# nmdp-bioinformatics/py-graph-imputation

Measured on AMD Instinct MI355X. Metric: imputed subjects/sec (whole node), 5-locus CAU graph, higher is better.
Workload: dtype f64; 1 GPU; BASELINE configs[1]: CAU 5-locus graph, 10k synthetic fully-typed subjects; 10000 subjects per step and GPU, seed=rank; graph_nodes=35411, populations=1

## Files before the change

### include/grim_hip.h

```cpp
#ifndef GRIM_HIP_H
#define GRIM_HIP_H

#include <stddef.h>
#include <stdint.h>

#ifdef __cplusplus
extern "C" {
#endif

#define GRIM_MAXL 5
#define GRIM_ABITS 12
#define GRIM_KEY_GRAPH_ORDER 60
#define GRIM_MAXPH 16
#define GRIM_MAXPOP 64
#define GRIM_TOPCAP 128
#define GRIM_MAXLADDER 64
#define GRIM_MAXROWS 8

typedef struct grim_ctx grim_ctx;
typedef struct grim_graph grim_graph;
typedef struct grim_batch grim_batch;

grim_ctx *grim_create(int device_id);
void grim_destroy(grim_ctx *ctx);
// ... 190 lines not shown
  const char *mask_ids;
  const uint8_t *mask_fixed;
  uint32_t n_masks;
} grim_stream_opts;

typedef struct {
  uint64_t lines, subjects, chunks, reruns;
  uint64_t unsupported;
  double wall_s;
  double tokenize_cpu_s, format_cpu_s, write_cpu_s;
  double device_s;
  double kernel_ms[7];
  uint64_t counters[4];
  uint64_t text_bytes[7];
  uint64_t bytes_h2d, bytes_d2h;
} grim_stream_stats;

grim_stream *grim_stream_open(grim_ctx *ctx, const grim_graph *g, const grim_dict *dict, const grim_params *prm,
                              const grim_prior_spec *priors, const char *const *pop_names, uint32_t n_pops,
                              const grim_stream_opts *opts);
int grim_stream_write(grim_stream *s, const char *text, uint64_t len);
int grim_stream_write_borrowed(grim_stream *s, const char *text, uint64_t len);
int grim_stream_write_text(grim_stream *s, const char *text, uint64_t len);
int grim_stream_write_file(grim_stream *s, const char *path);
int grim_stream_segment(grim_stream *s, uint64_t next_line_offset);
uint32_t grim_stream_n_segments(const grim_stream *s);
int grim_stream_segment_end(const grim_stream *s, uint32_t k, uint64_t out[7]);
int grim_stream_segment_wait(grim_stream *s, uint32_t k, uint64_t sizes[7]);
int grim_stream_segment_place(grim_stream *s, uint32_t k, const uint64_t base[6]);
int64_t grim_chunk_offsets(const char *path, uint32_t chunk_lines, uint64_t **out);
void grim_free(void *p);
uint32_t grim_default_threads(void);
int grim_stream_finish(grim_stream *s);
const char *grim_stream_error(const grim_stream *s);
const char *grim_stream_text(grim_stream *s, int which, uint64_t *len);
int grim_stream_get_stats(const grim_stream *s, grim_stream_stats *out);
int grim_stream_devtok_lines(const grim_stream *s, uint64_t *offered, uint64_t *handed_back);
uint32_t grim_tokname_hash(const char *name, uint32_t len);
uint64_t grim_stream_n_unsupported(const grim_stream *s);
int grim_stream_unsupported(const grim_stream *s, uint64_t k, uint64_t *line, uint32_t *reason, const char **id, uint32_t *id_len);
typedef struct {
  uint64_t first_line;
  uint32_t n_lines;
  const uint8_t *kinds;
  const grim_subject_result *res;
  const grim_row *rows;
  void *chunk;
// ... 108 lines not shown
```

### py-graph-imputation_amd/csrc/grim_engine.hip

```cpp
#include <hip/hip_runtime.h>
#include <hip/hip_ext.h>
#include <stdio.h>
#include <stdlib.h>
#include <string.h>
#include <algorithm>
#include <atomic>
#include <mutex>
#include <string>
#include <vector>

#include "grim_plan_a.h"
#include "grim_plan_b.h"
#include "grim_small.h"
#include "grim_medium.h"
#include "grim_mid.h"
#include "grim_tables.h"
#include "grim_tokdev.h"
#include "grim_em.h"
#include "grim_refresh.h"
#include "grim_marginal.h"
#include "grim_match.h"
#include "grim_search.h"
#include "grim_engine_internal.h"
#include "grim_host_internal.h"
// ... 1352 lines not shown
  }
  HIPCHK(hipEventRecord(b->ev_done, c->stream), c, -1);
  b->enqueued = true;
  return 0;
}

static int read_phase_times(grim_batch *b) {
  for (int p = 0; p < PH_COUNT; ++p)
    if (b->launched >> p & 1) HIPCHK(hipEventElapsedTime(&b->ms[p], b->ev[p][0], b->ev[p][1]), b->ctx, -1);
  b->launched = 0;
  return 0;
}

static inline uint32_t planb_count(const uint32_t *q) { return q[GRIM_Q_NEXT] + q[GRIM_Q_NEXT_HEAVY]; }

int engine_batch_wait(grim_batch *b) {
  if (!b) return -1;
  grim_ctx *c = b->ctx;
  use_device(c->device);
  DevArgs &A = b->a;
  if (!b->enqueued) {
    set_err(c, "engine_batch_wait: nothing in flight");
    return -1;
  }
  b->enqueued = false;
  b->ran_ok = false;
  HIPCHK(hipEventSynchronize(b->ev_done), c, -1);
  if (read_phase_times(b) != 0) return -1;
  uint32_t q[GRIM_NQ];
  auto read_queue = [&] { memcpy(q, b->hstate + GRIM_NCTR, sizeof(q)); };
  read_queue();
  const bool run_b = A.prm.planb && planb_count(q) > 0;
  if (run_b || stage2_pending(q) > 0) {
    {
      std::lock_guard<std::mutex> lk(c->run_mu);
      if (bind_scratch(b) != 0) return -1;
      if (run_b) {
        uint32_t grid = b->n_slots < planb_count(q) ? b->n_slots : planb_count(q);
        launch(b, PH_PLAN_B, grim_plan_b_kernel, dim3(grid), dim3(GRIM_WG), A);
        if (hipGetLastError() != hipSuccess) {
          set_err(c, "grim_batch_run: plan-B launch failed");
          return -1;
        }
      }
      enqueue_tables(b);
      launch(b, PH_NONE, grim_finish_kernel, dim3(1), dim3(GRIM_WG), A.counters, b->hstate, 0u, 1);
      HIPCHK(hipGetLastError(), c, -1);
      HIPCHK(hipEventRecord(b->ev_done, c->stream), c, -1);
    }
    HIPCHK(hipEventSynchronize(b->ev_done), c, -1);
    if (read_phase_times(b) != 0) return -1;
    read_queue();
  }
  if (b->timing) {
    for (int p = 0; p < PH_COUNT; ++p) b->acc_ms[p] += b->ms[p];
    b->n_timed++;
  }
  static const int dbg_classes = env_int("GRIM_DEBUG_CLASSES", 0);
  if (dbg_classes)
    fprintf(stderr, "grim classes: mid-size kernel took %u, handed %u to the general kernel\n"
            "grim classes: small %u medium %u general %u | medium->general %u (+%u heavier), to plan B %u (+%u heavy) | table items %u one-wave, %u bigger (%u work units), %u pair records; workgroup merge: %u items (%u with an overflowed bucket), up to %u pairs; workgroup split: %u items | stage 1 %s\n",
            q[GRIM_Q_MID_WORK], q[GRIM_Q_MID], b->n_small, b->n_medium, b->n_general, q[GRIM_Q_BAIL], q[GRIM_Q_BAIL_HEAVY], q[GRIM_Q_NEXT], q[GRIM_Q_NEXT_HEAVY], q[GRIM_Q_T1], q[GRIM_Q_T2],
            q[GRIM_Q_TUNITS], q[GRIM_Q_POOL], q[GRIM_Q_DBG_MERGE_WG], q[GRIM_Q_DBG_MERGE_OVF], q[GRIM_Q_DBG_MERGE_MAX], q[GRIM_Q_DBG_SPLIT_WG],
            b->graph_state == 1 ? "replayed as a hipGraph" : "launched directly");
  memcpy(b->counters, b->hstate, sizeof(b->counters));
// ... 157 lines not shown
  }();
  return on;
}
int engine_batch_fetch_issue(grim_batch *b) {
  if (!b) return -1;
  const bool ct = ct_on() != 0;
  if (ct) {
    b->ct_slot = (int)(g_ct_k.fetch_add(1) & 63);
    (void)hipEventRecord(g_ct_ev[0][b->ct_slot], b->ctx->copy_stream);
  }
  if (batch_fetch_on(b, 0, b->n_subj, nullptr, b->ctx->copy_stream, false) != 0) return -1;
  if (ct) (void)hipEventRecord(g_ct_ev[1][b->ct_slot], b->ctx->copy_stream);
  if (ct || !b->fetch_hsa) HIPCHK(hipEventRecord(b->ev_copy, b->ctx->copy_stream), b->ctx, -1);
  return 0;
}
int engine_batch_fetch_wait(grim_batch *b) {
  if (!b) return -1;
  use_device(b->ctx->device);
  if (b->fetch_hsa) {
    b->fetch_hsa = false;
    if (grim_sdma_wait(b->ctx->sdma, b->sdma_job) != 0) {
      set_err(b->ctx, "engine_batch_fetch: the SDMA copy of the results failed");
      return -1;
    }
    return 0;
  }
  HIPCHK(hipEventSynchronize(b->ev_copy), b->ctx, -1);
  if (ct_on() && b->ct_slot >= 0) {
    float ms = 0;
    if (hipEventElapsedTime(&ms, g_ct_ev[0][b->ct_slot], g_ct_ev[1][b->ct_slot]) == hipSuccess) { g_ct_ns += (uint64_t)(ms * 1e6); ++g_ct_n; }
    b->ct_slot = -1;
  }
  return 0;
}
extern "C" int grim_batch_results(grim_batch *b, grim_subject_result *res, grim_row *rows) {
  if (!b) return -1;
  grim_ctx *c = b->ctx;
  use_device(c->device);
  if (b->n_subj) HIPCHK(hipMemcpy(res, b->a.res, sizeof(grim_subject_result) * (size_t)b->n_subj, hipMemcpyDeviceToHost), c, -1);
  if (b->rows_used) HIPCHK(hipMemcpy(rows, b->a.rows, sizeof(grim_row) * (size_t)b->rows_used, hipMemcpyDeviceToHost), c, -1);
  return 0;
}
// ... 1302 lines not shown
```

### py-graph-imputation_amd/csrc/grim_engine_internal.h

```cpp
#pragma once
#include <stdint.h>

#include "../../include/grim_hip.h"
#include "grim_layout.h"
#include "grim_tok.h"

struct EnginePlan {
  uint32_t n_subj;
  uint64_t tok_cap;
  uint64_t text_cap;
};

struct EngineHost {
  grim_subject *subj;
  uint16_t *tok;
  SmallRec *small;
  uint32_t *order_s, *order_m, *order_g;
  grim_subject_result *res;
  grim_row *rows;
  LineRec *lines;
  uint8_t *text;
};

struct EngineLoad {
// ... 5 lines not shown
  uint32_t dev_lo, dev_hi;
  uint64_t text_bytes;
};

grim_batch *engine_batch_create(grim_ctx *ctx, const grim_graph *g, const grim_params *p, uint64_t row_limit, const EnginePlan *plan);
int engine_batch_plan(grim_batch *b, const EnginePlan *plan);
const EngineHost *engine_batch_host(grim_batch *b);
uint32_t engine_small_stride(const grim_params *p);
uint64_t engine_rows_per_subject(const grim_params *p, uint32_t n_pops);
int engine_batch_load(grim_batch *b, const EngineLoad *ld);
int engine_batch_fetch(grim_batch *b, uint32_t res_lo, uint32_t res_hi, grim_row *rows_dst);
uint64_t engine_bytes_moved(const grim_batch *b, int dir);
void engine_set_error(grim_ctx *ctx, const char *msg);
void engine_batch_recycle(grim_batch *b);
int engine_batch_fetch_issue(grim_batch *b);
int engine_batch_fetch_wait(grim_batch *b);
int engine_batch_upload_done(grim_batch *b);
int engine_batch_enqueue(grim_batch *b);
int engine_batch_wait(grim_batch *b);
struct DictSnap;
typedef struct grim_devdict grim_devdict;
grim_devdict *engine_devdict_create(grim_ctx *ctx, const DictSnap *snap);
void engine_devdict_free(grim_devdict *d);
void engine_batch_set_dict(grim_batch *b, const grim_devdict *d);
uint32_t engine_batch_irregular(const grim_batch *b);
uint32_t engine_graph_order_bad(const grim_graph *g);
uint64_t engine_batch_pool_want(const grim_batch *b);
void engine_batch_hint_pool(grim_batch *b, uint64_t records);
int engine_batch_grow_pool(grim_batch *b, uint64_t max_records);
int engine_batch_grow_rows(grim_batch *b, uint64_t max_rows);
uint64_t engine_batch_row_limit(const grim_batch *b);
void engine_batch_hint_rows(grim_batch *b, uint64_t rows);
```

### py-graph-imputation_amd/csrc/grim_host.cpp

```cpp
#include <stdint.h>
#include <stdlib.h>
#include <string.h>

#include <algorithm>
#include <charconv>
#include <cmath>
#include <mutex>
#include <string>
#include <string_view>
#include <thread>
#include <unordered_map>
#include <vector>

#include "../../include/grim_hip.h"

#include "grim_host_internal.h"

extern "C" grim_dict *grim_dict_create(uint32_t n_loci) {
  if (n_loci == 0 || n_loci > GRIM_MAXL) return nullptr;
  grim_dict *d = new grim_dict();
  d->n_loci = n_loci;
  d->locus_name.resize(n_loci);
  d->ids.resize(n_loci);
  d->names.resize(n_loci);
// ... 1113 lines not shown
  if (len) *len = t->t[which].size();
  return t->t[which].data();
}

extern "C" void grim_text_free(grim_text *t) { delete t; }

extern "C" int grim_format_double(double x, char *buf, int cap) {
  char b[48];
  char *e = py_float_to(x, b);
  const int n = (int)(e - b);
  if (n + 1 > cap) return -1;
  memcpy(buf, b, (size_t)n);
  buf[n] = 0;
  return n;
}
```

### py-graph-imputation_amd/csrc/grim_sdma.cpp

```cpp
#include "grim_sdma.h"

#include <hsa/hsa.h>
#include <hsa/hsa_ext_amd.h>
#include <stdio.h>
#include <stdlib.h>
#include <string.h>

#include <vector>

struct GrimSdma {
  hsa_agent_t gpu, cpu;
  hsa_amd_sdma_engine_id_t engine;
  uint64_t spin_ticks;
  uint32_t rec, avail;
  bool pinned_by_env;
};

namespace {
struct Agents {
  std::vector<hsa_agent_t> gpus, cpus;
};
hsa_status_t collect(hsa_agent_t a, void *data) {
  Agents *A = (Agents *)data;
  hsa_device_type_t t;
// ... 139 lines not shown
}

int grim_sdma_d2h_issue(GrimSdma *s, uint64_t job, void *dst_host, const void *src_dev, size_t bytes) {
  if (!s || !job) return -1;
  hsa_signal_t sig;
  sig.handle = job;
  hsa_signal_store_relaxed(sig, 1);
  const hsa_status_t st = hsa_amd_memory_async_copy_on_engine(dst_host, s->cpu, src_dev, s->gpu, bytes, 0, nullptr, sig, s->engine, true);
  if (st != HSA_STATUS_SUCCESS) {
    hsa_signal_store_relaxed(sig, 0);
    return -1;
  }
  return 0;
}

int grim_sdma_wait(GrimSdma *s, uint64_t job) {
  if (!s || !job) return -1;
  hsa_signal_t sig;
  sig.handle = job;
  hsa_signal_value_t v = hsa_signal_wait_scacquire(sig, HSA_SIGNAL_CONDITION_LT, 1, s->spin_ticks, HSA_WAIT_STATE_ACTIVE);
  while (v >= 1) v = hsa_signal_wait_scacquire(sig, HSA_SIGNAL_CONDITION_LT, 1, UINT64_MAX, HSA_WAIT_STATE_BLOCKED);
  return v < 0 ? -1 : 0;
}
```

### py-graph-imputation_amd/csrc/grim_sdma.h

```cpp
#pragma once
#include <stddef.h>
#include <stdint.h>

struct GrimSdma;

GrimSdma *grim_sdma_open(const char *hip_pci_bus_id, int hip_device_ordinal, const char **why);
void grim_sdma_close(GrimSdma *s);
uint32_t grim_sdma_engine(const GrimSdma *s);
uint32_t grim_sdma_pick(GrimSdma *s, void *dst_host, const void *src_dev, size_t bytes, char *report, size_t report_len);

int grim_sdma_job_create(GrimSdma *s, uint64_t *job);
void grim_sdma_job_destroy(GrimSdma *s, uint64_t job);
int grim_sdma_d2h_issue(GrimSdma *s, uint64_t job, void *dst_host, const void *src_dev, size_t bytes);
int grim_sdma_wait(GrimSdma *s, uint64_t job);
```

### py-graph-imputation_amd/csrc/grim_stream.cpp

```cpp
#include <errno.h>
#include <execinfo.h>
#include <fcntl.h>
#include <signal.h>
#include <sched.h>
#include <hip/hip_runtime_api.h>
#include <stdint.h>
#include <stdio.h>
#include <stdlib.h>
#include <string.h>
#include <sys/stat.h>
#include <sys/types.h>
#include <unistd.h>
#if defined(__x86_64__)
#include <immintrin.h>
#endif

#include <algorithm>
#include <atomic>
#include <chrono>
#include <condition_variable>
#include <deque>
#include <memory>
#include <mutex>
#include <string>
// ... 205 lines not shown
    char *dst = nullptr;
    size_t n = 0;
    std::vector<uint32_t> nl;
    uint32_t n_nl = 0;
  };
  std::vector<std::thread> copiers;
  std::vector<CopyJob> copy_jobs;
  std::atomic<uint64_t> copy_ticket{0}, copy_np_gen{0};
  std::mutex copy_mu;
  std::condition_variable cv_copyjob;
  std::atomic<uint64_t> copy_gen{0};
  std::atomic<int> copy_left{0};
  bool copy_stop = false;
  uint32_t avg_line = 128;
  std::thread dev_thread, copy_thread, fetch_thread;
  std::deque<Chunk *> copy_q, fetch_q;
  std::condition_variable cv_copy, cv_fetch;
  uint64_t next_device = 0, next_commit = 0, next_record = 0, n_done = 0;

  int fd[6] = {-1, -1, -1, -1, -1, -1};
  uint64_t file_pos[7] = {0, 0, 0, 0, 0, 0, 0};
  std::vector<std::pair<char *, size_t>> mem[7];
  std::string joined[7];
  bool joined_ok[7] = {false, false, false, false, false, false, false};

  struct Unsup {
    uint64_t line;
    uint32_t reason;
    std::string id;
  };
// ... 317 lines not shown
    Chunk *c = nullptr;
    {
      std::unique_lock<std::mutex> lk(s->mu);
      for (;;) {
        if (s->stop || s->failed) return;
        c = s->by_index(s->next_device);
        if (c && c->state == CH_TOKENIZED) break;
        c = nullptr;
        if (loaded) break;
        s->cv_dev.wait(lk);
      }
      if (c) ++s->next_device;
    }
    if (!c && loaded && !eager) {
      const auto w0 = Clock::now();
      for (int spin = 0;; ++spin) {
        if (engine_batch_upload_done(loaded->batch)) break;
        if ((spin & 7) == 7) {
          if (secs(w0, Clock::now()) > 200e-6) break;
          std::unique_lock<std::mutex> lk(s->mu, std::try_to_lock);
          if (lk.owns_lock()) {
            if (s->stop || s->failed) return;
            Chunk *n = s->by_index(s->next_device);
            if (n && n->state == CH_TOKENIZED) {
              c = n;
              ++s->next_device;
              break;
            }
          }
        }
// ... 33 lines not shown
      Chunk *l = loaded;
      loaded = nullptr;
      if (!launch(l, 0)) return;
    }
    if (c) {
      if (c->n_dev_subjects && rc == 0) {
        loaded = c;
      } else if (!launch(c, rc)) {
        return;
      }
    }
  }
}

static void copy_loop(grim_stream *s) {
  for (;;) {
    Chunk *c = nullptr;
    {
      std::unique_lock<std::mutex> lk(s->mu);
      for (;;) {
        if (s->stop || s->failed) return;
        if (!s->copy_q.empty()) {
          c = s->copy_q.front();
          s->copy_q.pop_front();
          break;
        }
        s->cv_copy.wait(lk);
      }
    }
    const auto t0 = Clock::now();
    int rc = 0;
    PartStats ps;
    if (c->n_dev_subjects) {
      if (c->in_flight) {
        c->in_flight = false;
        const int wrc = engine_batch_wait(c->batch);
        tl_note(c, 5);
        auto lb = [](const std::vector<uint32_t> &v, uint32_t x) { return (size_t)(std::lower_bound(v.begin(), v.end(), x) - v.begin()); };
        const size_t rng[4] = {0, lb(c->os, c->n_lines), 0, lb(c->om, c->n_lines)};
        rc = finish_part(s, c, 0, c->n_lines, true, wrc, rng, (uint32_t)c->og_sorted.size(), ps);
      } else {
        rc = device_part_sync(s, c, 0, c->n_lines, true, ps);
      }
      if (rc == 0 && !c->extra_rows.empty()) c->rows = c->extra_rows.data();
    }
    const auto t1 = Clock::now();
    g_dbg_ns[2] += (uint64_t)(secs(t0, t1) * 1e9);
    bool issued = false, fetched_ok = true;
    if (rc == 0 && c->n_dev_subjects && c->fetch_pending && c->extra_rows.empty()) {
      fetched_ok = engine_batch_fetch_issue(c->batch) == 0;
      issued = fetched_ok;
// ... 10 lines not shown
        s->fail(std::string(rc != 0 ? "device stage failed: " : "device stage failed: copying the results to the host: ") + (e ? e : ""));
        return;
      }
      if (issued) {
        s->fetch_q.push_back(c);
        s->cv_fetch.notify_all();
      } else {
        c->state = CH_DEVICE_DONE;
      }
    }
    if (!issued) enqueue_format(s, c);
  }
}

static void fetch_loop(grim_stream *s) {
  for (;;) {
    Chunk *c = nullptr;
    {
      std::unique_lock<std::mutex> lk(s->mu);
      for (;;) {
        if (s->stop || s->failed) return;
        if (!s->fetch_q.empty()) {
          c = s->fetch_q.front();
          s->fetch_q.pop_front();
          break;
        }
        s->cv_fetch.wait(lk);
      }
    }
    const auto t0 = Clock::now();
    const bool ok = engine_batch_fetch_wait(c->batch) == 0;
    tl_note(c, 7);
    g_dbg_ns[3] += (uint64_t)(secs(t0, Clock::now()) * 1e9);
    {
      std::lock_guard<std::mutex> lk(s->mu);
      if (!ok) {
        const char *e = grim_last_error(s->ctx);
        s->fail(std::string("device stage failed: copying the results to the host: ") + (e ? e : ""));
        return;
      }
      c->rows = engine_batch_host(c->batch)->rows;
      c->state = CH_DEVICE_DONE;
    }
    enqueue_format(s, c);
  }
}
// ... 223 lines not shown
  uint32_t k = 0;
  for (size_t i = 0; i < n; ++i) {
    dst[i] = src[i];
    if (src[i] == '\n') nl[k++] = (uint32_t)i;
  }
  return k;
}

static constexpr size_t COPY_PIECES = 64;
static void copy_pieces(grim_stream *s) {
  for (;;) {
    const uint64_t t = s->copy_ticket.fetch_add(1, std::memory_order_acq_rel);
    const uint64_t ng = s->copy_np_gen.load(std::memory_order_acquire);
    const uint32_t k = (uint32_t)t;
    if ((ng >> 32) != (t >> 32) || k >= (uint32_t)ng) return;
    grim_stream::CopyJob &job = s->copy_jobs[k];
    tl_dbg[0] = k; tl_dbg[1] = (uint64_t)job.dst; tl_dbg[2] = (uint64_t)job.src; tl_dbg[3] = job.n; tl_dbg[4] = (uint64_t)job.nl.data();
    tl_dbg[5] = job.nl.size(); tl_dbg[6] = t; tl_dbg[7] = ng;
    job.n_nl = copy_and_mark(job.dst, job.src, job.n, job.nl.data());
    s->copy_left.fetch_sub(1, std::memory_order_release);
  }
}

static void copier_loop(grim_stream *s, size_t) {
  uint64_t seen = 0;
  for (;;) {
    {
      uint64_t gen = s->copy_gen.load(std::memory_order_acquire);
      if (gen == seen) {
        const auto t0 = Clock::now();
        for (int spin = 0; gen == seen; ++spin) {
          if ((spin & 63) == 63 && secs(t0, Clock::now()) > 250e-6) break;
#if defined(__x86_64__)
          __builtin_ia32_pause();
#endif
          gen = s->copy_gen.load(std::memory_order_acquire);
        }
      }
      if (gen == seen) {
        std::unique_lock<std::mutex> lk(s->copy_mu);
        s->cv_copyjob.wait(lk, [&] { return s->copy_stop || s->copy_gen.load(std::memory_order_acquire) != seen; });
        if (s->copy_stop) return;
        gen = s->copy_gen.load(std::memory_order_acquire);
      }
      seen = gen;
    }
    copy_pieces(s);
  }
}

static Chunk *acquire_chunk(grim_stream *s) {
  std::unique_lock<std::mutex> lk(s->mu);
// ... 245 lines not shown
        for (size_t k = 0; k < parts; ++k) {
          const size_t o = std::min<size_t>(blk, k * per), e = std::min<size_t>(blk, (k + 1) * per);
          grim_stream::CopyJob &j = s->copy_jobs[k];
          j.src = text + a + o;
          j.dst = as_view ? nullptr : c->text.data() + base + o;
          j.n = e - o;
          j.n_nl = 0;
          if (j.nl.size() < j.n + 64) j.nl.resize(j.n + 64);
        }
        const uint64_t blk_no = (s->copy_gen.load(std::memory_order_relaxed) + 1) & 0xFFFFFFFFull;
        s->copy_np_gen.store(blk_no << 32 | (uint64_t)parts, std::memory_order_release);
        s->copy_left.store((int)parts);
        s->copy_ticket.store(blk_no << 32, std::memory_order_release);
        s->copy_gen.fetch_add(1, std::memory_order_release);
      }
      s->cv_copyjob.notify_all();
      copy_pieces(s);
      while (s->copy_left.load(std::memory_order_acquire) > 0) std::this_thread::yield();
      const auto tr2 = Clock::now();
      g_dbg_ns[8] += (uint64_t)(secs(tr1, tr2) * 1e9);
      used = blk;
      bool full = false;
      for (size_t q = 0; q < parts && !full; ++q) {
        const grim_stream::CopyJob &j = s->copy_jobs[q];
        const uint64_t po = std::min<size_t>(blk, q * per);
        const uint32_t take = std::min<uint32_t>(j.n_nl, want - got);
        uint32_t ln = c->n_lines + got;
        uint32_t first = s->granule - ln % s->granule;
        for (uint32_t i = first; i <= take; i += s->granule)
          if (ln + i < s->chunk_lines) c->mark_off.push_back(base + po + j.nl[i - 1] + 1);
        got += take;
// ... 201 lines not shown
  }
  if (len) *len = s->joined[which].size();
  return s->joined[which].data();
}

extern "C" int grim_stream_get_stats(const grim_stream *s, grim_stream_stats *out) {
  if (!s || !out) return -1;
  {
    std::lock_guard<std::mutex> lk(const_cast<grim_stream *>(s)->mu);
    *out = s->st;
  }
  out->tokenize_cpu_s = s->tok_ns.load() * 1e-9;
  out->format_cpu_s = s->fmt_ns.load() * 1e-9;
  out->write_cpu_s = s->wr_ns.load() * 1e-9;
  out->unsupported = s->unsupported.size();
  out->bytes_h2d = engine_bytes_moved(nullptr, 0);
  out->bytes_d2h = engine_bytes_moved(nullptr, 1);
  return 0;
}

extern "C" int grim_stream_devtok_lines(const grim_stream *s, uint64_t *offered, uint64_t *handed_back) {
  if (!s) return -1;
  if (offered) *offered = s->offered.load();
  if (handed_back) *handed_back = s->handed_back.load();
  return 0;
}

extern "C" uint64_t grim_stream_n_unsupported(const grim_stream *s) { return s ? s->unsupported.size() : 0; }

extern "C" int grim_stream_unsupported(const grim_stream *s, uint64_t k, uint64_t *line, uint32_t *reason, const char **id, uint32_t *id_len) {
// ... 31 lines not shown
  }
}

extern "C" int grim_stream_release_records(grim_stream *s, grim_stream_records *rec) {
  if (!s || !rec || !rec->chunk) return -1;
  Chunk *c = (Chunk *)rec->chunk;
  std::lock_guard<std::mutex> lk(s->mu);
  c->records_released = true;
  tl_note(c, 9);
  tl_close(c);
  rec->chunk = nullptr;
  release_if_done(s, c);
  return 0;
}

extern "C" uint32_t grim_default_threads(void) {
  unsigned cores = 0;
  cpu_set_t set;
  CPU_ZERO(&set);
  if (sched_getaffinity(0, sizeof(set), &set) == 0) cores = (unsigned)CPU_COUNT(&set);
  if (!cores) cores = std::max(1u, std::thread::hardware_concurrency());
  unsigned ranks = 1;
  const char *lw = getenv("LOCAL_WORLD_SIZE");
  if (!lw || atoi(lw) <= 0) lw = getenv("WORLD_SIZE");
  if (lw && atoi(lw) > 0) ranks = (unsigned)atoi(lw);
  unsigned nt = cores / ranks;
  if (nt < 1) nt = 1;
  if (nt > 32) nt = 32;
  return nt;
}

static void segv_backtrace(int sig, siginfo_t *si, void *) {
  void *frames[48];
  const int n = backtrace(frames, 48);
  char buf[512];
  const int m = snprintf(buf, sizeof(buf), "grim: SIGSEGV at address %p; copy job: k=%llu dst=%llx src=%llx n=%llu nl=%llx nl_size=%llu ticket=%llx np_gen=%llx\n"
                         "native frames of the faulting thread:\n", si ? si->si_addr : nullptr, (unsigned long long)tl_dbg[0], (unsigned long long)tl_dbg[1],
                         (unsigned long long)tl_dbg[2], (unsigned long long)tl_dbg[3], (unsigned long long)tl_dbg[4], (unsigned long long)tl_dbg[5],
                         (unsigned long long)tl_dbg[6], (unsigned long long)tl_dbg[7]);
  (void)!write(2, buf, (size_t)m);
  backtrace_symbols_fd(frames, n, 2);
  signal(sig, SIG_DFL);
// ... 49 lines not shown
      p += n + 1;
    }
    s->have_masks = true;
  } else if (opts->mask_ids) {
    s->have_masks = true;
  }
  s->rule.small_ok = (n_pops == 1) && prm->opt_threshold > 1 && !getenv("GRIM_NO_SMALL") && engine_graph_order_bad(g) == 0;
  s->rule.medium_ok = !getenv("GRIM_NO_MEDIUM") && engine_graph_order_bad(g) == 0;
  s->rule.medium_max_cost = getenv("GRIM_MEDIUM_MAXCOST") ? atof(getenv("GRIM_MEDIUM_MAXCOST")) : 0.0;
  s->rule.graph_loci = s->snap.n_loci;
  s->rule.opt_threshold = prm->opt_threshold;
  s->chunk_lines = opts->chunk_lines ? opts->chunk_lines : 131072u;
  s->granule = 1024;
  if (s->chunk_lines < s->granule) s->granule = s->chunk_lines;
  s->depth = opts->depth ? opts->depth : 4u;
  int nt = opts->n_threads;
  if (nt <= 0) nt = (int)grim_default_threads();
  s->n_threads = (uint32_t)nt;
  const uint64_t per = engine_rows_per_subject(prm, n_pops);
  uint64_t rows = opts->rows_per_chunk ? opts->rows_per_chunk : 32ull * s->chunk_lines;
  const uint64_t floor_rows = 2ull * engine_small_stride(prm) * s->chunk_lines + 2 * per + 4 * 64 + 1024;
  if (rows < floor_rows && !(opts->rows_exact && opts->rows_per_chunk)) rows = floor_rows;
  if (rows > 0x7FFFFFF0ull) rows = 0x7FFFFFF0ull;
  s->rows_per_chunk = rows;
  s->rows_max = opts->rows_per_chunk ? 0 : std::max<uint64_t>(rows, std::min<uint64_t>(0x7FFFFFF0ull, floor_rows + per * s->chunk_lines));
  {
    const char *e = getenv("GRIM_DEVICE_TOKENIZER");
    s->dev_tok = s->rule.small_ok && !s->have_masks && s->snap.n_loci == GRIM_MAXL && !(e && atoi(e) == 0);
    if (s->dev_tok) {
      s->devdict = engine_devdict_create(ctx, &s->snap);
      if (!s->devdict) {
        delete s;
        return nullptr;
// ... 37 lines not shown
        return nullptr;
      }
    }
  for (auto &pr : parked) s->stale.push_back(pr.first);
  if (!s->stale.empty())
    s->unlinker = std::thread([s]() {
      for (const std::string &f : s->stale) unlink(f.c_str());
    });
  s->t_open = Clock::now();
  for (uint32_t i = 0; i < s->n_threads; ++i) s->workers.emplace_back(worker_loop, s);
  s->dev_thread = std::thread(device_loop, s);
  s->copy_thread = std::thread(copy_loop, s);
  s->fetch_thread = std::thread(fetch_loop, s);
  {
    const char *e = getenv("GRIM_COPY_THREADS");
    size_t nc = e ? (size_t)atoi(e) : (s->n_threads >= 24 ? 7u : s->n_threads >= 12 ? 5u : s->n_threads >= 8 ? 3u : s->n_threads >= 4 ? 1u : 0u);
    if (nc > 7) nc = 7;
    s->copy_jobs.resize(COPY_PIECES);
    for (size_t k = 0; k < nc; ++k) s->copiers.emplace_back(copier_loop, s, k);
  }
  return s;
}

extern "C" void grim_stream_free(grim_stream *s) {
  if (!s) return;
  if (getenv("GRIM_DEBUG_STREAM"))
    fprintf(stderr, "grim stream: device thread ms: staging %.3f load %.3f | copy thread ms: wait + stage 2 %.3f fetch %.3f | reader ms: work %.3f "
            "(copy %.3f scan %.3f dispatch %.3f) waiting for a slot %.3f | consumer waiting %.3f over %llu chunks\n", g_dbg_ns[0] / 1e6, g_dbg_ns[1] / 1e6, g_dbg_ns[2] / 1e6,
            g_dbg_ns[3] / 1e6, g_dbg_ns[4] / 1e6, g_dbg_ns[8] / 1e6, g_dbg_ns[9] / 1e6, g_dbg_ns[7] / 1e6, g_dbg_ns[5] / 1e6, g_dbg_ns[6] / 1e6, (unsigned long long)s->st.chunks);
  if (getenv("GRIM_DEBUG_STREAM") && g_tl_n.load()) {
    static const char *nm[10] = {"", "fill", "tokenise", "-> device thread", "load + launch", "-> kernels done", "stage 2 + export issued", "-> on the host", "-> consumer", "consumer"};
// ... 38 lines not shown
```

### py-graph-imputation_amd/grim/_native.py

```python

import ctypes as C
import os

import numpy as np

MAXL = 5
ABITS = 12
MAXPH = 16
MAXPOP = 64
TOPCAP = 128
MAXLADDER = 64
MAXROWS = 8

ST_OK, ST_MISS, ST_UNSUPPORTED, ST_NOPHASE = 0, 1, 2, 3
T_UMUG, T_UMUG_POPS, T_PMUG, T_PMUG_POPS = 0, 1, 2, 3
(MS_TOTAL, MS_PLAN_A, MS_PLAN_B, MS_HALF_WAVE, MS_GENERAL, MS_ONE_WAVE, MS_TABLES, MS_COMPACT, MS_TOKENIZER,
 MS_MID) = range(10)
MS_MEAN = 0x10

_HERE = os.path.dirname(os.path.abspath(__file__))
LIB_PATH = os.environ.get("GRIM_LIB") or os.path.join(os.path.dirname(_HERE), "libgrim_hip.so")


class GraphDesc(C.Structure):
# ... 757 lines not shown
    _fields_ = [("alpha", C.c_double), ("eta", C.c_double), ("beta", C.c_double), ("gamma", C.c_double), ("delta", C.c_double),
                ("unk_mr", C.c_uint8), ("count_by_prob", C.POINTER(C.c_double))]


class StreamOpts(C.Structure):
    _fields_ = [("chunk_lines", C.c_uint32), ("depth", C.c_uint32), ("n_threads", C.c_int32), ("line_offset", C.c_uint64),
                ("rows_per_chunk", C.c_uint64), ("want_text", C.c_uint8), ("want_log", C.c_uint8), ("want_records", C.c_uint8),
                ("timing", C.c_uint8), ("rows_exact", C.c_uint8), ("placed", C.c_uint8), ("out_path", C.c_char_p * 6), ("mask_ids", C.c_char_p), ("mask_fixed", C.c_void_p),
                ("n_masks", C.c_uint32)]


class StreamStats(C.Structure):
    _fields_ = [("lines", C.c_uint64), ("subjects", C.c_uint64), ("chunks", C.c_uint64), ("reruns", C.c_uint64),
                ("unsupported", C.c_uint64), ("wall_s", C.c_double), ("tokenize_cpu_s", C.c_double), ("format_cpu_s", C.c_double),
                ("write_cpu_s", C.c_double), ("device_s", C.c_double), ("kernel_ms", C.c_double * 7), ("counters", C.c_uint64 * 4),
                ("text_bytes", C.c_uint64 * 7), ("bytes_h2d", C.c_uint64), ("bytes_d2h", C.c_uint64)]


class StreamRecords(C.Structure):
    _fields_ = [("first_line", C.c_uint64), ("n_lines", C.c_uint32), ("kinds", C.c_void_p), ("res", C.c_void_p),
                ("rows", C.c_void_p), ("chunk", C.c_void_p)]


_host_ready = False


def host_lib():
    global _host_ready
    L = lib()
    if _host_ready:
        return L
# ... 92 lines not shown
    L.grim_stream_n_segments.argtypes = [C.c_void_p]
    L.grim_stream_segment_end.restype = C.c_int
    L.grim_stream_segment_end.argtypes = [C.c_void_p, C.c_uint32, C.POINTER(C.c_uint64)]
    L.grim_stream_segment_wait.restype = C.c_int
    L.grim_stream_segment_wait.argtypes = [C.c_void_p, C.c_uint32, C.POINTER(C.c_uint64)]
    L.grim_stream_segment_place.restype = C.c_int
    L.grim_stream_segment_place.argtypes = [C.c_void_p, C.c_uint32, C.POINTER(C.c_uint64)]
    L.grim_stream_devtok_lines.restype = C.c_int
    L.grim_stream_devtok_lines.argtypes = [C.c_void_p, C.POINTER(C.c_uint64), C.POINTER(C.c_uint64)]
    L.grim_tokname_hash.restype = C.c_uint32
    L.grim_tokname_hash.argtypes = [C.c_char_p, C.c_uint32]
    L.grim_default_threads.restype = C.c_uint32
    L.grim_chunk_offsets.restype = C.c_int64
    L.grim_chunk_offsets.argtypes = [C.c_char_p, C.c_uint32, C.POINTER(C.POINTER(C.c_uint64))]
    L.grim_free.argtypes = [C.c_void_p]
    _host_ready = True
    return L


def tokname_hash(name):
    b = name.encode() if isinstance(name, str) else bytes(name)
    return int(host_lib().grim_tokname_hash(b, len(b)))


def host_threads():
    n = int(os.environ.get("GRIM_HOST_THREADS", "0"))
    if n <= 0:
        n = min(16, os.cpu_count() or 1)
    return n


class AlleleDict:
# ... 362 lines not shown
```

Measured before the change: 148.9 million subjects/s.

## Budget host CPUs from cgroups and cap spinning waiters to avoid oversubscription

Adds cgroup-aware CPU budget detection (cpu.max, CFS quota, GRIM_HOST_CPUS) and uses it to size worker and copy-helper threads, reserving cores for the service threads. Limits how many threads may busy-spin on GPU events and SDMA signals at once; the rest poll with nanosleep or block. Copier wakeups now chain through notify_one instead of notify_all, and the wait threads lower their timer slack. The goal is to stop spinning threads from starving workers on constrained hosts, at the cost of added wake-up latency for threads that sleep.

After: 201.3 million subjects/s, median of 6. +35.1%, better.

```diff
diff --git a/include/grim_hip.h b/include/grim_hip.h
--- a/include/grim_hip.h
+++ b/include/grim_hip.h
@@ -228,6 +228,8 @@
   uint64_t counters[4];
   uint64_t text_bytes[7];
   uint64_t bytes_h2d, bytes_d2h;
+  uint32_t workers, copy_helpers, spin_places, reserved;
+  uint64_t waits_spun, waits_asleep;
 } grim_stream_stats;
 
 grim_stream *grim_stream_open(grim_ctx *ctx, const grim_graph *g, const grim_dict *dict, const grim_params *prm,
@@ -245,6 +247,9 @@
 int64_t grim_chunk_offsets(const char *path, uint32_t chunk_lines, uint64_t **out);
 void grim_free(void *p);
 uint32_t grim_default_threads(void);
+uint32_t grim_cpu_budget(void);
+uint32_t grim_cpu_budget_from(uint32_t affinity_cpus, const char *cpu_max, const char *cfs_quota_us, const char *cfs_period_us,
+                              const char *host_cpus);
 int grim_stream_finish(grim_stream *s);
 const char *grim_stream_error(const grim_stream *s);
 const char *grim_stream_text(grim_stream *s, int which, uint64_t *len);
diff --git a/py-graph-imputation_amd/csrc/grim_engine.hip b/py-graph-imputation_amd/csrc/grim_engine.hip
--- a/py-graph-imputation_amd/csrc/grim_engine.hip
+++ b/py-graph-imputation_amd/csrc/grim_engine.hip
@@ -3,6 +3,7 @@
 #include <stdio.h>
 #include <stdlib.h>
 #include <string.h>
+#include <time.h>
 #include <algorithm>
 #include <atomic>
 #include <mutex>
@@ -1390,7 +1391,18 @@
 
 static inline uint32_t planb_count(const uint32_t *q) { return q[GRIM_Q_NEXT] + q[GRIM_Q_NEXT_HEAVY]; }
 
-int engine_batch_wait(grim_batch *b) {
+static hipError_t wait_event(hipEvent_t ev, bool spin) {
+  if (spin) return hipEventSynchronize(ev);
+  for (;;) {
+    const hipError_t e = hipEventQuery(ev);
+    if (e != hipErrorNotReady) return e;
+    (void)hipGetLastError();
+    struct timespec ts = {0, 20000};
+    nanosleep(&ts, nullptr);
+  }
+}
+
+int engine_batch_wait(grim_batch *b, bool spin) {
   if (!b) return -1;
   grim_ctx *c = b->ctx;
   use_device(c->device);
@@ -1401,7 +1413,7 @@
   }
   b->enqueued = false;
   b->ran_ok = false;
-  HIPCHK(hipEventSynchronize(b->ev_done), c, -1);
+  HIPCHK(wait_event(b->ev_done, spin), c, -1);
   if (read_phase_times(b) != 0) return -1;
   uint32_t q[GRIM_NQ];
   auto read_queue = [&] { memcpy(q, b->hstate + GRIM_NCTR, sizeof(q)); };
@@ -1424,7 +1436,7 @@
       HIPCHK(hipGetLastError(), c, -1);
       HIPCHK(hipEventRecord(b->ev_done, c->stream), c, -1);
     }
-    HIPCHK(hipEventSynchronize(b->ev_done), c, -1);
+    HIPCHK(wait_event(b->ev_done, spin), c, -1);
     if (read_phase_times(b) != 0) return -1;
     read_queue();
   }
@@ -1612,18 +1624,18 @@
   if (ct || !b->fetch_hsa) HIPCHK(hipEventRecord(b->ev_copy, b->ctx->copy_stream), b->ctx, -1);
   return 0;
 }
-int engine_batch_fetch_wait(grim_batch *b) {
+int engine_batch_fetch_wait(grim_batch *b, bool spin) {
   if (!b) return -1;
   use_device(b->ctx->device);
   if (b->fetch_hsa) {
     b->fetch_hsa = false;
-    if (grim_sdma_wait(b->ctx->sdma, b->sdma_job) != 0) {
+    if (grim_sdma_wait(b->ctx->sdma, b->sdma_job, spin) != 0) {
       set_err(b->ctx, "engine_batch_fetch: the SDMA copy of the results failed");
       return -1;
     }
     return 0;
   }
-  HIPCHK(hipEventSynchronize(b->ev_copy), b->ctx, -1);
+  HIPCHK(wait_event(b->ev_copy, spin), b->ctx, -1);
   if (ct_on() && b->ct_slot >= 0) {
     float ms = 0;
     if (hipEventElapsedTime(&ms, g_ct_ev[0][b->ct_slot], g_ct_ev[1][b->ct_slot]) == hipSuccess) { g_ct_ns += (uint64_t)(ms * 1e6); ++g_ct_n; }
diff --git a/py-graph-imputation_amd/csrc/grim_engine_internal.h b/py-graph-imputation_amd/csrc/grim_engine_internal.h
--- a/py-graph-imputation_amd/csrc/grim_engine_internal.h
+++ b/py-graph-imputation_amd/csrc/grim_engine_internal.h
@@ -43,10 +43,10 @@
 void engine_set_error(grim_ctx *ctx, const char *msg);
 void engine_batch_recycle(grim_batch *b);
 int engine_batch_fetch_issue(grim_batch *b);
-int engine_batch_fetch_wait(grim_batch *b);
+int engine_batch_fetch_wait(grim_batch *b, bool spin = true);
 int engine_batch_upload_done(grim_batch *b);
 int engine_batch_enqueue(grim_batch *b);
-int engine_batch_wait(grim_batch *b);
+int engine_batch_wait(grim_batch *b, bool spin = true);
 struct DictSnap;
 typedef struct grim_devdict grim_devdict;
 grim_devdict *engine_devdict_create(grim_ctx *ctx, const DictSnap *snap);
diff --git a/py-graph-imputation_amd/csrc/grim_host.cpp b/py-graph-imputation_amd/csrc/grim_host.cpp
--- a/py-graph-imputation_amd/csrc/grim_host.cpp
+++ b/py-graph-imputation_amd/csrc/grim_host.cpp
@@ -1151,3 +1151,44 @@
   buf[n] = 0;
   return n;
 }
+
+static uint32_t quota_cpus(long long quota, long long period) {
+  if (quota <= 0 || period <= 0) return 0;
+  const long long c = (quota + period - 1) / period;
+  return (uint32_t)std::min<long long>(std::max<long long>(c, 1), 1 << 20);
+}
+static bool parse_ll(const char *&p, long long &out) {
+  while (*p == ' ' || *p == '\t' || *p == '\n' || *p == '\r') ++p;
+  char *e = nullptr;
+  const long long v = strtoll(p, &e, 10);
+  if (e == p) return false;
+  p = e;
+  out = v;
+  return true;
+}
+static uint32_t cpu_max_cpus(const char *t) {
+  if (!t) return 0;
+  long long q = 0, per = 0;
+  if (!parse_ll(t, q) || !parse_ll(t, per)) return 0;
+  return quota_cpus(q, per);
+}
+extern "C" uint32_t grim_cpu_budget_from(uint32_t affinity_cpus, const char *cpu_max, const char *cfs_quota_us, const char *cfs_period_us,
+                                         const char *host_cpus) {
+  uint32_t b = affinity_cpus ? affinity_cpus : 0xFFFFFFFFu;
+  auto take = [&](uint32_t c) {
+    if (c && c < b) b = c;
+  };
+  take(cpu_max_cpus(cpu_max));
+  if (cfs_quota_us && cfs_period_us) {
+    long long q = 0, per = 0;
+    const char *a = cfs_quota_us, *c = cfs_period_us;
+    if (parse_ll(a, q) && parse_ll(c, per)) take(quota_cpus(q, per));
+  }
+  if (host_cpus) {
+    long long h = 0;
+    const char *a = host_cpus;
+    if (parse_ll(a, h) && h > 0) take((uint32_t)std::min<long long>(h, 1 << 20));
+  }
+  if (b == 0xFFFFFFFFu) b = std::max(1u, std::thread::hardware_concurrency());
+  return b;
+}
diff --git a/py-graph-imputation_amd/csrc/grim_sdma.cpp b/py-graph-imputation_amd/csrc/grim_sdma.cpp
--- a/py-graph-imputation_amd/csrc/grim_sdma.cpp
+++ b/py-graph-imputation_amd/csrc/grim_sdma.cpp
@@ -177,11 +177,12 @@
   return 0;
 }
 
-int grim_sdma_wait(GrimSdma *s, uint64_t job) {
+int grim_sdma_wait(GrimSdma *s, uint64_t job, bool spin) {
   if (!s || !job) return -1;
   hsa_signal_t sig;
   sig.handle = job;
-  hsa_signal_value_t v = hsa_signal_wait_scacquire(sig, HSA_SIGNAL_CONDITION_LT, 1, s->spin_ticks, HSA_WAIT_STATE_ACTIVE);
+  hsa_signal_value_t v = spin ? hsa_signal_wait_scacquire(sig, HSA_SIGNAL_CONDITION_LT, 1, s->spin_ticks, HSA_WAIT_STATE_ACTIVE)
+                              : hsa_signal_load_scacquire(sig);
   while (v >= 1) v = hsa_signal_wait_scacquire(sig, HSA_SIGNAL_CONDITION_LT, 1, UINT64_MAX, HSA_WAIT_STATE_BLOCKED);
   return v < 0 ? -1 : 0;
 }
diff --git a/py-graph-imputation_amd/csrc/grim_sdma.h b/py-graph-imputation_amd/csrc/grim_sdma.h
--- a/py-graph-imputation_amd/csrc/grim_sdma.h
+++ b/py-graph-imputation_amd/csrc/grim_sdma.h
@@ -12,4 +12,4 @@
 int grim_sdma_job_create(GrimSdma *s, uint64_t *job);
 void grim_sdma_job_destroy(GrimSdma *s, uint64_t job);
 int grim_sdma_d2h_issue(GrimSdma *s, uint64_t job, void *dst_host, const void *src_dev, size_t bytes);
-int grim_sdma_wait(GrimSdma *s, uint64_t job);
+int grim_sdma_wait(GrimSdma *s, uint64_t job, bool spin = true);
diff --git a/py-graph-imputation_amd/csrc/grim_stream.cpp b/py-graph-imputation_amd/csrc/grim_stream.cpp
--- a/py-graph-imputation_amd/csrc/grim_stream.cpp
+++ b/py-graph-imputation_amd/csrc/grim_stream.cpp
@@ -8,6 +8,7 @@
 #include <stdio.h>
 #include <stdlib.h>
 #include <string.h>
+#include <sys/prctl.h>
 #include <sys/stat.h>
 #include <sys/types.h>
 #include <unistd.h>
@@ -243,6 +244,22 @@
   bool copy_stop = false;
   uint32_t avg_line = 128;
   std::thread dev_thread, copy_thread, fetch_thread;
+  std::atomic<int> spinning{0};
+  int spin_cap = 1;
+  uint32_t cpu_budget = 1;
+  bool spin_enter() {
+    int v = spinning.load(std::memory_order_relaxed);
+    while (v < spin_cap)
+      if (spinning.compare_exchange_weak(v, v + 1, std::memory_order_relaxed)) return true;
+    return false;
+  }
+  void spin_leave() { spinning.fetch_sub(1, std::memory_order_relaxed); }
+  std::atomic<uint64_t> waits_spun{0}, waits_asleep{0};
+  bool spin_or_sleep() {
+    const bool spin = spin_enter();
+    (spin ? waits_spun : waits_asleep).fetch_add(1, std::memory_order_relaxed);
+    return spin;
+  }
   std::deque<Chunk *> copy_q, fetch_q;
   std::condition_variable cv_copy, cv_fetch;
   uint64_t next_device = 0, next_commit = 0, next_record = 0, n_done = 0;
@@ -590,6 +607,11 @@
     }
     if (!c && loaded && !eager) {
       const auto w0 = Clock::now();
+      struct Counted {
+        grim_stream *s;
+        explicit Counted(grim_stream *s_) : s(s_) { s->spinning.fetch_add(1, std::memory_order_relaxed); }
+        ~Counted() { s->spin_leave(); }
+      } counted(s);
       for (int spin = 0;; ++spin) {
         if (engine_batch_upload_done(loaded->batch)) break;
         if ((spin & 7) == 7) {
@@ -653,6 +675,7 @@
 }
 
 static void copy_loop(grim_stream *s) {
+  prctl(PR_SET_TIMERSLACK, 1000UL, 0UL, 0UL, 0UL);
   for (;;) {
     Chunk *c = nullptr;
     {
@@ -673,7 +696,9 @@
     if (c->n_dev_subjects) {
       if (c->in_flight) {
         c->in_flight = false;
-        const int wrc = engine_batch_wait(c->batch);
+        const bool spin = s->spin_or_sleep();
+        const int wrc = engine_batch_wait(c->batch, spin);
+        if (spin) s->spin_leave();
         tl_note(c, 5);
         auto lb = [](const std::vector<uint32_t> &v, uint32_t x) { return (size_t)(std::lower_bound(v.begin(), v.end(), x) - v.begin()); };
         const size_t rng[4] = {0, lb(c->os, c->n_lines), 0, lb(c->om, c->n_lines)};
@@ -714,6 +739,7 @@
 }
 
 static void fetch_loop(grim_stream *s) {
+  prctl(PR_SET_TIMERSLACK, 1000UL, 0UL, 0UL, 0UL);
   for (;;) {
     Chunk *c = nullptr;
     {
@@ -729,7 +755,9 @@
       }
     }
     const auto t0 = Clock::now();
-    const bool ok = engine_batch_fetch_wait(c->batch) == 0;
+    const bool spin = s->spin_or_sleep();
+    const bool ok = engine_batch_fetch_wait(c->batch, spin) == 0;
+    if (spin) s->spin_leave();
     tl_note(c, 7);
     g_dbg_ns[3] += (uint64_t)(secs(t0, Clock::now()) * 1e9);
     {
@@ -983,6 +1011,7 @@
     const uint64_t ng = s->copy_np_gen.load(std::memory_order_acquire);
     const uint32_t k = (uint32_t)t;
     if ((ng >> 32) != (t >> 32) || k >= (uint32_t)ng) return;
+    if (k + 1 < (uint32_t)ng) s->cv_copyjob.notify_one();
     grim_stream::CopyJob &job = s->copy_jobs[k];
     tl_dbg[0] = k; tl_dbg[1] = (uint64_t)job.dst; tl_dbg[2] = (uint64_t)job.src; tl_dbg[3] = job.n; tl_dbg[4] = (uint64_t)job.nl.data();
     tl_dbg[5] = job.nl.size(); tl_dbg[6] = t; tl_dbg[7] = ng;
@@ -996,7 +1025,7 @@
   for (;;) {
     {
       uint64_t gen = s->copy_gen.load(std::memory_order_acquire);
-      if (gen == seen) {
+      if (gen == seen && s->spin_or_sleep()) {
         const auto t0 = Clock::now();
         for (int spin = 0; gen == seen; ++spin) {
           if ((spin & 63) == 63 && secs(t0, Clock::now()) > 250e-6) break;
@@ -1005,6 +1034,7 @@
 #endif
           gen = s->copy_gen.load(std::memory_order_acquire);
         }
+        s->spin_leave();
       }
       if (gen == seen) {
         std::unique_lock<std::mutex> lk(s->copy_mu);
@@ -1280,7 +1310,7 @@
         s->copy_ticket.store(blk_no << 32, std::memory_order_release);
         s->copy_gen.fetch_add(1, std::memory_order_release);
       }
-      s->cv_copyjob.notify_all();
+      s->cv_copyjob.notify_one();
       copy_pieces(s);
       while (s->copy_left.load(std::memory_order_acquire) > 0) std::this_thread::yield();
       const auto tr2 = Clock::now();
@@ -1512,6 +1542,12 @@
   out->format_cpu_s = s->fmt_ns.load() * 1e-9;
   out->write_cpu_s = s->wr_ns.load() * 1e-9;
   out->unsupported = s->unsupported.size();
+  out->workers = s->n_threads;
+  out->copy_helpers = (uint32_t)s->copiers.size();
+  out->spin_places = (uint32_t)s->spin_cap;
+  out->reserved = 0;
+  out->waits_spun = s->waits_spun.load();
+  out->waits_asleep = s->waits_asleep.load();
   out->bytes_h2d = engine_bytes_moved(nullptr, 0);
   out->bytes_d2h = engine_bytes_moved(nullptr, 1);
   return 0;
@@ -1573,18 +1609,72 @@
   return 0;
 }
 
-extern "C" uint32_t grim_default_threads(void) {
+static bool read_small_file(const std::string &path, std::string &out) {
+  out.clear();
+  const int fd = open(path.c_str(), O_RDONLY);
+  if (fd < 0) return false;
+  char buf[256];
+  const ssize_t n = read(fd, buf, sizeof(buf) - 1);
+  close(fd);
+  if (n <= 0) return false;
+  out.assign(buf, (size_t)n);
+  return true;
+}
+
+extern "C" uint32_t grim_cpu_budget(void) {
   unsigned cores = 0;
   cpu_set_t set;
   CPU_ZERO(&set);
   if (sched_getaffinity(0, sizeof(set), &set) == 0) cores = (unsigned)CPU_COUNT(&set);
-  if (!cores) cores = std::max(1u, std::thread::hardware_concurrency());
+  uint32_t b = grim_cpu_budget_from(cores, nullptr, nullptr, nullptr, getenv("GRIM_HOST_CPUS"));
+  std::string cg, txt, txt2;
+  const int fd = open("/proc/self/cgroup", O_RDONLY);
+  if (fd >= 0) {
+    char buf[4096];
+    ssize_t n;
+    while ((n = read(fd, buf, sizeof(buf))) > 0) cg.append(buf, (size_t)n);
+    close(fd);
+  }
+  std::vector<std::string> v2_paths{""}, v1_paths{""};
+  for (size_t a = 0; a < cg.size();) {
+    size_t e = cg.find('\n', a);
+    if (e == std::string::npos) e = cg.size();
+    const std::string line = cg.substr(a, e - a);
+    a = e + 1;
+    const size_t c1 = line.find(':'), c2 = c1 == std::string::npos ? c1 : line.find(':', c1 + 1);
+    if (c2 == std::string::npos) continue;
+    const std::string ctl = line.substr(c1 + 1, c2 - c1 - 1);
+    std::string path = line.substr(c2 + 1);
+    if (path.find("..") != std::string::npos) continue;
+    const bool v2 = ctl.empty();
+    if (!v2 && ("," + ctl + ",").find(",cpu,") == std::string::npos) continue;
+    while (path.size() > 1) {
+      (v2 ? v2_paths : v1_paths).push_back(path);
+      const size_t up = path.rfind('/');
+      if (up == std::string::npos) break;
+      path.erase(up);
+    }
+  }
+  for (const std::string &p : v2_paths)
+    if (read_small_file("/sys/fs/cgroup" + p + "/cpu.max", txt)) b = grim_cpu_budget_from(b, txt.c_str(), nullptr, nullptr, nullptr);
+  for (const char *mnt : {"/sys/fs/cgroup/cpu", "/sys/fs/cgroup/cpu,cpuacct"})
+    for (const std::string &p : v1_paths)
+      if (read_small_file(std::string(mnt) + p + "/cpu.cfs_quota_us", txt) && read_small_file(std::string(mnt) + p + "/cpu.cfs_period_us", txt2))
+        b = grim_cpu_budget_from(b, nullptr, txt.c_str(), txt2.c_str(), nullptr);
+  return b ? b : 1;
+}
+
+static unsigned local_ranks() {
   unsigned ranks = 1;
   const char *lw = getenv("LOCAL_WORLD_SIZE");
   if (!lw || atoi(lw) <= 0) lw = getenv("WORLD_SIZE");
   if (lw && atoi(lw) > 0) ranks = (unsigned)atoi(lw);
-  unsigned nt = cores / ranks;
-  if (nt < 1) nt = 1;
+  return ranks;
+}
+
+extern "C" uint32_t grim_default_threads(void) {
+  const unsigned share = grim_cpu_budget() / local_ranks();
+  unsigned nt = share > 5 ? share - 5 : 1;
   if (nt > 32) nt = 32;
   return nt;
 }
@@ -1664,9 +1754,11 @@
   s->granule = 1024;
   if (s->chunk_lines < s->granule) s->granule = s->chunk_lines;
   s->depth = opts->depth ? opts->depth : 4u;
+  s->cpu_budget = std::max(1u, grim_cpu_budget() / local_ranks());
   int nt = opts->n_threads;
   if (nt <= 0) nt = (int)grim_default_threads();
   s->n_threads = (uint32_t)nt;
+  s->spin_cap = (int)std::max(1u, s->cpu_budget / 8);
   const uint64_t per = engine_rows_per_subject(prm, n_pops);
   uint64_t rows = opts->rows_per_chunk ? opts->rows_per_chunk : 32ull * s->chunk_lines;
   const uint64_t floor_rows = 2ull * engine_small_stride(prm) * s->chunk_lines + 2 * per + 4 * 64 + 1024;
@@ -1734,7 +1826,8 @@
   s->fetch_thread = std::thread(fetch_loop, s);
   {
     const char *e = getenv("GRIM_COPY_THREADS");
-    size_t nc = e ? (size_t)atoi(e) : (s->n_threads >= 24 ? 7u : s->n_threads >= 12 ? 5u : s->n_threads >= 8 ? 3u : s->n_threads >= 4 ? 1u : 0u);
+    const uint32_t cb = s->cpu_budget;
+    size_t nc = e ? (size_t)atoi(e) : (cb >= 48 ? 7u : cb >= 24 ? 5u : cb >= 12 ? 3u : cb >= 4 ? 1u : 0u);
     if (nc > 7) nc = 7;
     s->copy_jobs.resize(COPY_PIECES);
     for (size_t k = 0; k < nc; ++k) s->copiers.emplace_back(copier_loop, s, k);
diff --git a/py-graph-imputation_amd/grim/_native.py b/py-graph-imputation_amd/grim/_native.py
--- a/py-graph-imputation_amd/grim/_native.py
+++ b/py-graph-imputation_amd/grim/_native.py
@@ -795,7 +795,9 @@
     _fields_ = [("lines", C.c_uint64), ("subjects", C.c_uint64), ("chunks", C.c_uint64), ("reruns", C.c_uint64),
                 ("unsupported", C.c_uint64), ("wall_s", C.c_double), ("tokenize_cpu_s", C.c_double), ("format_cpu_s", C.c_double),
                 ("write_cpu_s", C.c_double), ("device_s", C.c_double), ("kernel_ms", C.c_double * 7), ("counters", C.c_uint64 * 4),
-                ("text_bytes", C.c_uint64 * 7), ("bytes_h2d", C.c_uint64), ("bytes_d2h", C.c_uint64)]
+                ("text_bytes", C.c_uint64 * 7), ("bytes_h2d", C.c_uint64), ("bytes_d2h", C.c_uint64),
+                ("workers", C.c_uint32), ("copy_helpers", C.c_uint32), ("spin_places", C.c_uint32), ("reserved", C.c_uint32),
+                ("waits_spun", C.c_uint64), ("waits_asleep", C.c_uint64)]
 
 
 class StreamRecords(C.Structure):
@@ -918,8 +920,19 @@
     L.grim_chunk_offsets.restype = C.c_int64
     L.grim_chunk_offsets.argtypes = [C.c_char_p, C.c_uint32, C.POINTER(C.POINTER(C.c_uint64))]
     L.grim_free.argtypes = [C.c_void_p]
+    L.grim_cpu_budget.restype = C.c_uint32
+    L.grim_cpu_budget_from.restype = C.c_uint32
+    L.grim_cpu_budget_from.argtypes = [C.c_uint32, C.c_char_p, C.c_char_p, C.c_char_p, C.c_char_p]
     _host_ready = True
     return L
+
+
+EXPORTS += ["grim_cpu_budget", "grim_cpu_budget_from"]
+
+
+def cpu_budget_from(affinity, cpu_max=None, cfs_quota=None, cfs_period=None, host_cpus=None):
+    enc = lambda t: None if t is None else (t.encode() if isinstance(t, str) else bytes(t))
+    return int(host_lib().grim_cpu_budget_from(int(affinity), enc(cpu_max), enc(cfs_quota), enc(cfs_period), enc(host_cpus)))
 
 
 def tokname_hash(name):
```
